# hammershock/SFM-Python

Hardware: AMD Instinct MI355X
Metric: BA iterations/sec (higher is better)
Workload: dtype f64

## Files before the change

sfm-python_amd/csrc/ba_kernels.hpp:

```cpp
#pragma once

#include <hip/hip_runtime.h>
#include <stdint.h>

#include "tr2d.hpp"

namespace sfmba {

constexpr int kCamTab = 17;
constexpr int kCamRow = 18;
#ifndef SFMBA_REC_LAYOUT
#define SFMBA_REC_LAYOUT 0
#endif
constexpr int kRecLayout = SFMBA_REC_LAYOUT;
constexpr int kRec = kRecLayout == 0 ? 6 : (kRecLayout == 1 ? 8 : 16);
constexpr int kVinvRow = kRecLayout == 0 ? 6 : (kRecLayout == 1 ? 8 : 16);
constexpr int kVinvInRec = kRecLayout == 2 ? 8 : -1;
constexpr int kRhsRec = 16;
constexpr int kSweepThreads = 1024;
constexpr int kWavesPerSweepBlock = kSweepThreads / 64;

struct KMat { double k[9]; };

constexpr int kJPlanes = 6;
// ... 2995 lines not shown
    }
    const size_t n6 = 6 * (size_t)C;
    const int set = ci.iters & 1;
    const double* __restrict__ vin = vecs + (size_t)set * kPcgVecs * n6;
    double* __restrict__ vout = vecs + (size_t)(set ^ 1) * kPcgVecs * n6;
    const double* __restrict__ u_in = vin + kPcgU * n6;
    const int slice = ((C + (int)gridDim.x - 1) / (int)gridDim.x + 63) & ~63;
    const int own_lo = (int)blockIdx.x * slice, own_hi = own_lo + slice;

    double d[1] = {0.0};
    for (int c = threadIdx.x; c < C; c += blockDim.x) {
#pragma unroll
        for (int k = 0; k < 6; ++k) {
            const size_t e = (size_t)k * C + c;
            const double ue = u_in[e];
            d[0] += (acc_in[e] + Dc[e] * ue) * ue;
        }
    }
    block_sum<1>(d, red);
    if (threadIdx.x == 0) sh_bcast[0] = d[0];
    __syncthreads();
    const double delta = sh_bcast[0];
    const double gamma = ci.rz;
    const double beta = ci.iters == 0 ? 0.0 : gamma / ci.rz_prev;
    const double den = delta - (ci.iters == 0 ? 0.0 : beta * gamma / ci.alpha_prev);
    const double alpha = gamma / den;
    if (!(den > 0.0) || !isfinite(alpha)) {
        if (blockIdx.x == 0 && threadIdx.x == 0) { PcgCtrl co = ci; co.done = 3; *cout = co; }
        return;
    }
    double t[1] = {0.0};
    for (int c = threadIdx.x; c < C; c += blockDim.x) {
        double rr[6], uu[6], pp[6], ss[6], xx[6], m[21];
#pragma unroll
        for (int n = 0; n < 21; ++n) m[n] = Minv[(size_t)n * C + c];
#pragma unroll
        for (int k = 0; k < 6; ++k) {
            const size_t e = (size_t)k * C + c;
            const double ue = u_in[e];
            const double we = acc_in[e] + Dc[e] * ue;
            pp[k] = ue + beta * vin[kPcgP * n6 + e];
            ss[k] = we + beta * vin[kPcgS * n6 + e];
            xx[k] = vin[kPcgX * n6 + e] + alpha * pp[k];
            rr[k] = vin[kPcgR * n6 + e] - alpha * ss[k];
        }
#pragma unroll
        for (int k = 0; k < 6; ++k) {
            uu[k] = minv_row(m, rr, k);
            t[0] += uu[k] * rr[k];
        }
        if (c >= own_lo && c < own_hi) {
#pragma unroll
            for (int k = 0; k < 6; ++k) {
                const size_t e = (size_t)k * C + c;
                vout[kPcgX * n6 + e] = xx[k]; vout[kPcgR * n6 + e] = rr[k];
                vout[kPcgP * n6 + e] = pp[k]; vout[kPcgS * n6 + e] = ss[k];
                vout[kPcgU * n6 + e] = uu[k];
                vout[kPcgUcm * n6 + 6 * (size_t)c + k] = uu[k];
            }
        }
    }
    block_sum<1>(t, red);
    if (blockIdx.x == 0 && threadIdx.x == 0) {
        PcgCtrl co = ci;
        co.rz_prev = ci.rz;
        co.alpha_prev = alpha;
        co.rz = t[0];
        co.iters = ci.iters + 1;
        if (!(t[0] > ci.tol2 * ci.rz0)) co.done = 1;
        else if (co.iters >= ci.max_iters) co.done = 2;
        *cout = co;
    }
}

constexpr int kBacksubCols = 10;
struct FinalUpdate {
    const double* __restrict__ part;
    double* __restrict__ vecs;
    PcgCtrl* __restrict__ ctrl2;
    int L;
};
template <bool LDS_VEC, bool JFREE = false>
__global__ __launch_bounds__(kSweepThreads) void k_backsub(
    const int2* __restrict__ ranges, int n_ranges, ObsArrays o, const double* __restrict__ dc_planes,
    double* __restrict__ dc, const double* __restrict__ Vinv, const double* __restrict__ gp,
    const double* __restrict__ t1, double* __restrict__ dp, double* __restrict__ part, int C,
    const PcgCtrl* __restrict__ ctrl2, int L, const double* __restrict__ gvec,
    const double* __restrict__ si, const double* __restrict__ sg, Recompute rc, FinalUpdate fu) {
    static_assert(!(LDS_VEC && JFREE), "J-free: the LDS holds the camera table, the step vector comes from L2");
    extern __shared__ __align__(16) double smem[];
    __shared__ double red[kBacksubCols * kWavesPerSweepBlock];
    if (LDS_VEC && fu.part != nullptr) {
        const int n6 = 6 * C, cam = threadIdx.x;
        const PcgCtrl ci = fu.ctrl2[fu.L & 1];
        PcgCtrl co = ci;
        double alpha = 0.0;
        double xe[6] = {0.0, 0.0, 0.0, 0.0, 0.0, 0.0}, pe[6] = {0.0, 0.0, 0.0, 0.0, 0.0, 0.0};
        if (cam < C) {
#pragma unroll
            for (int k = 0; k < 6; ++k) {
                xe[k] = fu.vecs[kPcgX * n6 + (size_t)k * C + cam];
                pe[k] = fu.vecs[kPcgP * n6 + (size_t)k * C + cam];
            }
        }
        if (ci.done == 0) alpha = pcg_local_step(fu.part, C, ci, co);
        if (blockIdx.x == 0 && threadIdx.x == 0) fu.ctrl2[(fu.L + 1) & 1] = co;
        if (co.done == 0) return;
        const bool add = ci.done == 0 && co.done != 3;
        if (cam < C) {
#pragma unroll
            for (int k = 0; k < 6; ++k) {
                const double xk = add ? xe[k] + alpha * pe[k] : xe[k];
                smem[6 * cam + k] = xk;
                if (blockIdx.x == 0) dc[6 * cam + k] = xk;
            }
        }
        __syncthreads();
    } else {
    if (ctrl2 != nullptr)
        dc_planes += (size_t)((ctrl2[L & 1].iters & 1) * kPcgVecs + kPcgX) * 6 * C;
    if (LDS_VEC) {
        for (int i = threadIdx.x; i < 6 * C; i += blockDim.x) {
            const int k = i / C, c = i - k * C;
            const double val = dc_planes[i];
            smem[6 * c + k] = val;
            if (blockIdx.x == 0) dc[6 * c + k] = val;
        }
        __syncthreads();
    }
    }
    if (JFREE) stage_cam_table(rc.camtab, C, smem);
    const double* __restrict__ vv = LDS_VEC ? smem : dc;
    const int wg = blockIdx.x * (blockDim.x >> 6) + (threadIdx.x >> 6);
    const int lane = threadIdx.x & 63;
    int pos = 0, end = 0;
    if (wg < n_ranges) { const int2 rg = ranges[wg]; pos = rg.x; end = rg.y; }
    auto blocks_of = [&](int j, int pj, double* jc_, double* jp_) {
        if (JFREE) recompute_blocks(rc, smem, o.cam_idx[j], pj, jc_, jp_);
        else load_blocks(o, j, jc_, jp_);
    };
    double g12 = 0.0, g22 = 0.0;
    double qs[8] = {0.0, 0.0, 0.0, 0.0, 0.0, 0.0, 0.0, 0.0};
    auto dots = [&](double* q, size_t e, double pe) {
        const double s = si[e];
        q[0] += gvec[e] * pe; q[1] += (pe * s) * (pe * s); q[2] += sg[e] * pe; q[3] += pe * pe;
    };

    auto jcv = [&](const double* jc, int c, double& t0, double& t1v) {
        const double2* a2 = reinterpret_cast<const double2*>(vv + 6 * c);
        const double2 a01 = a2[0], a23 = a2[1], a45 = a2[2];
        const double a[6] = {a01.x, a01.y, a23.x, a23.y, a45.x, a45.y};
        t0 = 0.0; t1v = 0.0;
#pragma unroll
        for (int k = 0; k < 6; ++k) { t0 += jc[k] * a[k]; t1v += jc[6 + k] * a[k]; }
    };
    auto point_dots = [&](int p, const double* s3, double z0, double z1, double z2) {
        const double z[3] = {z0, z1, z2};
#pragma unroll
        for (int k = 0; k < 3; ++k) {
            const double s_ = s3[k], ge = gp[3 * (size_t)p + k], pe = z[k];
            qs[0] += ge * pe; qs[1] += (pe * s_) * (pe * s_); qs[2] += (ge / (s_ * s_)) * pe; qs[3] += pe * pe;
        }
    };
    auto solve_point = [&](int p, const double* y, double& z0, double& z1, double& z2) {
        const double* vi = Vinv + kVinvRow * (size_t)p;
        const double b0 = -gp[3 * (size_t)p] - y[0], b1 = -gp[3 * (size_t)p + 1] - y[1],
                     b2 = -gp[3 * (size_t)p + 2] - y[2];
        z0 = vi[0] * b0 + vi[1] * b1 + vi[2] * b2;
        z1 = vi[1] * b0 + vi[3] * b1 + vi[4] * b2;
        z2 = vi[2] * b0 + vi[4] * b1 + vi[5] * b2;
        dp[3 * (size_t)p] = z0; dp[3 * (size_t)p + 1] = z1; dp[3 * (size_t)p + 2] = z2;
    };
    auto gram = [&](int i, const double* jp, double t0, double t1v, double z0, double z1, double z2) {
        const double a0 = t0 + jp[0] * z0 + jp[1] * z1 + jp[2] * z2;
        const double a1 = t1v + jp[3] * z0 + jp[4] * z1 + jp[5] * z2;
        const double2 tt = load_pair(t1, o.f32, i);
        g12 += tt.x * a0 + tt.y * a1;
        g22 += a0 * a0 + a1 * a1;
    };

    while (pos < end) {
        const int i = pos + lane;
        const bool in = i < end;
        const int p = in ? o.pt_idx[i] : o.pt_idx[pos];
        const int sb = o.pt_ptr[p], se = o.pt_ptr[p + 1];
        const bool complete = in && (se <= pos + 64);
        const int n_take = __popcll(__ballot(complete));
        double jc[12], jp[6];
        if (n_take == 0) {
            const int run_end = __shfl(se, 0);
            const int pp = __shfl(p, 0);
            double y[3] = {0.0, 0.0, 0.0};
            for (int j = pos + lane; j < run_end; j += 64) {
                blocks_of(j, pp, jc, jp);
                double t0, t1v;
                jcv(jc, o.cam_idx[j], t0, t1v);
                y[0] += jp[0] * t0 + jp[3] * t1v; y[1] += jp[1] * t0 + jp[4] * t1v;
                y[2] += jp[2] * t0 + jp[5] * t1v;
            }
            y[0] = wave_sum(y[0]); y[1] = wave_sum(y[1]); y[2] = wave_sum(y[2]);
            double z0, z1, z2;
            solve_point(pp, y, z0, z1, z2);
            if (lane == 0) point_dots(pp, si + 6 * (size_t)C + 3 * (size_t)pp, z0, z1, z2);
            for (int j = pos + lane; j < run_end; j += 64) {
                blocks_of(j, pp, jc, jp);
                double t0, t1v;
                jcv(jc, o.cam_idx[j], t0, t1v);
                gram(j, jp, t0, t1v, z0, z1, z2);
            }
            pos = run_end;
            continue;
        }
        const bool act = lane < n_take;
        double t0 = 0.0, t1v = 0.0, z0 = 0.0, z1 = 0.0, z2 = 0.0;
        double y[3] = {0.0, 0.0, 0.0};
        double s3[3] = {1.0, 1.0, 1.0};
        if (act) {
            blocks_of(i, p, jc, jp);
#pragma unroll
            for (int k = 0; k < 3; ++k) s3[k] = si[6 * (size_t)C + 3 * (size_t)p + k];
            jcv(jc, o.cam_idx[i], t0, t1v);
            y[0] = jp[0] * t0 + jp[3] * t1v; y[1] = jp[1] * t0 + jp[4] * t1v;
            y[2] = jp[2] * t0 + jp[5] * t1v;
        }
        seg_reduce_serial<3>(y, act ? sb : -1 - lane, lane);
        if (act && i == sb) { solve_point(p, y, z0, z1, z2); point_dots(p, s3, z0, z1, z2); }
        const int head = act ? lane - (i - sb) : lane;
        z0 = __shfl(z0, head); z1 = __shfl(z1, head); z2 = __shfl(z2, head);
        if (act) gram(i, jp, t0, t1v, z0, z1, z2);
        pos += n_take;
    }
    {
        const int per = (6 * C + (int)gridDim.x - 1) / (int)gridDim.x;
        const int e = (int)blockIdx.x * per + (int)threadIdx.x;
        if ((int)threadIdx.x < per && e < 6 * C) dots(qs + 4, (size_t)e, vv[e]);
    }
    double row[kBacksubCols];
    row[0] = wave_sum(g12);
    row[1] = wave_sum(g22);
#pragma unroll
    for (int k = 0; k < 8; ++k) row[2 + k] = wave_sum(qs[k]);
    if (lane == 0) {
#pragma unroll
        for (int k = 0; k < kBacksubCols; ++k) red[kBacksubCols * (threadIdx.x >> 6) + k] = row[k];
    }
    __syncthreads();
    if (threadIdx.x < kBacksubCols) {
        double a = 0.0;
        for (int w = 0; w < (int)(blockDim.x >> 6); ++w) a += red[kBacksubCols * w + threadIdx.x];
        part[(size_t)kBacksubCols * blockIdx.x + threadIdx.x] = a;
    }
}

__global__ void k_transpose(const double* __restrict__ in, int rows, int cols, double* __restrict__ out,
                            const PcgCtrl* __restrict__ ctrl2, int L) {
    const int i = blockIdx.x * blockDim.x + threadIdx.x;
    if (i >= rows * cols) return;
    if (ctrl2 != nullptr) in += (size_t)((ctrl2[L & 1].iters & 1) * kPcgVecs + kPcgX) * rows * cols;
    const int r = i / cols, c = i - r * cols;
    out[(size_t)c * rows + r] = in[i];
}

constexpr int kP2pMaxRanks = 16;
constexpr int kP2pFlagStride = 16;
constexpr int kP2pMaxBlocks = 32;
struct P2pArgs {
    double* data[kP2pMaxRanks];
    unsigned long long* flags[kP2pMaxRanks];
    int rank, world;
    long long stride;
    unsigned long long* seq;
    const int* cancel;
    unsigned* ticket;
    unsigned* error;
    long long timeout;
    unsigned long long max_mask;
    Piggyback rider;
    Mailbox post;
    const double* skip;
};

#ifdef SFMBA_P2P_NOFENCE
#ifndef SFMBA_EXPERIMENT
#error "SFMBA_P2P_NOFENCE builds collectives that are formally unordered: measurement builds only (-DSFMBA_EXPERIMENT)"
#endif
#define P2P_FENCE() asm volatile("s_waitcnt vmcnt(0) lgkmcnt(0)" ::: "memory")
#else
#define P2P_FENCE() __threadfence_system()
#endif
__device__ __forceinline__ unsigned p2p_take_ticket(unsigned* ticket) {
    return __hip_atomic_fetch_add(ticket, 1u, __ATOMIC_ACQ_REL, __HIP_MEMORY_SCOPE_AGENT);
}
__device__ __forceinline__ void p2p_allreduce_body(double* __restrict__ vec, int count, int op, const P2pArgs& a) {
    __shared__ unsigned s_last;
    const int tid = threadIdx.x;
    const unsigned long long seq = *a.seq + 1ull;
    const int par = (int)(seq & 1ull);
    const int per = (count + (int)gridDim.x - 1) / (int)gridDim.x;
    const int lo = (int)blockIdx.x * per, hi = min(count, lo + per);
    for (int q = 0; q < a.world; ++q) {
        double* dst = a.data[q] + ((size_t)par * a.world + a.rank) * a.stride;
        for (int e = lo + tid; e < hi; e += blockDim.x)
            __hip_atomic_store(dst + e, vec[e], __ATOMIC_RELAXED, __HIP_MEMORY_SCOPE_SYSTEM);
    }
    P2P_FENCE();
    __syncthreads();
    if (tid == 0) s_last = (p2p_take_ticket(a.ticket) == gridDim.x - 1) ? 1u : 0u;
    __syncthreads();
    if (s_last != 0u) {
        if (tid < a.world)
            __hip_atomic_store(a.flags[tid] + ((size_t)par * a.world + a.rank) * kP2pFlagStride, seq,
                               __ATOMIC_RELEASE, __HIP_MEMORY_SCOPE_SYSTEM);
        if (tid == 0) { *a.ticket = 0u; *a.seq = seq; }
// ... 156 lines not shown
```

sfm-python_amd/csrc/sfmba.hip:

```cpp
#include "../../include/sfmba.h"

#include <hip/hip_runtime.h>
#include <hip/hip_ext.h>
#include <rccl/rccl.h>
#include <dlfcn.h>

#include <algorithm>
#include <atomic>
#include <chrono>
#include <cmath>
#include <cstdarg>
#include <cstdio>
#include <cstdlib>
#include <cstring>
#include <condition_variable>
#include <functional>
#include <mutex>
#include <numeric>
#include <string>
#include <thread>
#include <vector>

#include "ba_kernels.hpp"
#include "tr2d.hpp"
// ... 96 lines not shown
            std::function<void(int)>* f = nullptr;
            {
                std::unique_lock<std::mutex> lk(m_);
                cv_.wait(lk, [&] { return gen_ != seen; });
                seen = gen_;
                if (stop_) return;
                if (id >= job_parts_ || job_ == nullptr) continue;
                f = job_;
            }
            (*f)(id);
            {
                std::lock_guard<std::mutex> lk(m_);
                if (--pending_ == 0) done_.notify_one();
            }
        }
    }
    std::vector<std::thread> th_;
    std::mutex m_;
    std::condition_variable cv_, done_;
    std::function<void(int)>* job_ = nullptr;
    int job_parts_ = 0, pending_ = 0;
    unsigned long long gen_ = 0;
    bool stop_ = false;
};

struct RcclApi {
    void* lib = nullptr;
    ncclResult_t (*GetUniqueId)(ncclUniqueId*) = nullptr;
    ncclResult_t (*CommInitRank)(ncclComm_t*, int, ncclUniqueId, int) = nullptr;
    ncclResult_t (*AllReduce)(const void*, void*, size_t, ncclDataType_t, ncclRedOp_t, ncclComm_t, hipStream_t) = nullptr;
    ncclResult_t (*CommDestroy)(ncclComm_t) = nullptr;
    const char* (*GetErrorString)(ncclResult_t) = nullptr;
};
RcclApi* rccl_api() {
    static RcclApi api;
    static bool tried = false;
    if (!tried) {
        tried = true;
        void* lib = dlopen("librccl.so.1", RTLD_NOW | RTLD_GLOBAL);
        if (!lib) lib = dlopen("librccl.so", RTLD_NOW | RTLD_GLOBAL);
        if (!lib) lib = dlopen("/opt/rocm/lib/librccl.so.1", RTLD_NOW | RTLD_GLOBAL);
        if (lib) {
            api.GetUniqueId = (decltype(api.GetUniqueId))dlsym(lib, "ncclGetUniqueId");
            api.CommInitRank = (decltype(api.CommInitRank))dlsym(lib, "ncclCommInitRank");
            api.AllReduce = (decltype(api.AllReduce))dlsym(lib, "ncclAllReduce");
            api.CommDestroy = (decltype(api.CommDestroy))dlsym(lib, "ncclCommDestroy");
            api.GetErrorString = (decltype(api.GetErrorString))dlsym(lib, "ncclGetErrorString");
            if (api.GetUniqueId && api.CommInitRank && api.AllReduce && api.CommDestroy && api.GetErrorString)
                api.lib = lib;
        }
    }
    return api.lib ? &api : nullptr;
}

double now_s() {
    return std::chrono::duration<double>(std::chrono::steady_clock::now().time_since_epoch()).count();
}

}

struct sfmba_handle {
    int device = 0;
    hipStream_t stream = nullptr;
    bool own_stream = false;
    std::string err;
    int n_cu = 256;

    bool have_problem = false;
    int64_t C = 0, P = 0, N = 0, ld = 0, n = 0;
    int64_t N_total = 0;
    KMat K{};
    bool permuted = false;
    std::vector<int64_t> order;
    int n_ranges = 0;
    bool f32 = false;
    bool f32_next = false;
    std::vector<int64_t> fixed_next;
    int64_t n_fixed = 0;
    bool lds_tab = true, lds_vec = true;
    bool sweep_rc = false;
    bool sweep_rc_g = false;
    DevBuf rctab;
    bool jfree = false;
    bool mixed = false;
    bool mixed_b = false;
    DevBuf rt32, rec32, rctab32, rtd;
    Origin origin{0.0, 0.0, 0.0};
    bool dense = false;
    DevView cov_ptr, cov_pt, blk_ab;
    DevBuf Sblk;
    DevBuf tables;
    int n_blk = 0;
    struct Debug {
        int pcg_fused = -1;
        int tab_lds = -1, vec_lds = -1;
        int sweep_rc = -1;
        int dense = -1;
        int precond = -1;
        int pcg_local = -1;
        int xcd_chunks = -1;
        int rhsrec = -1;
        int cost_rider = -1;
        int packed_upload = -1;
        int jfree = -1;
        int cm_device = -1;
        int pcg_inline = -1;
        int xcd_cam = -1;
        int pcg_skip_last = -1;
        int pcg_mixed_b = -1;
        int pcg_mixed = -1;
        int pcg_split = -1;
        int cam_chunk = 0;
        int pcg_guess_bias = 0;
        int trace_pcg = 0, trace_stalls = 0, trace_timing = 0;
        int wait_deadline_s = 120;
        int p2p_delay_ms = 0;
        int p2p_timeout_ms = 0;
    } dbg;

    DevBuf cam_idx, pt_idx, pt_ptr, uv;
    DevView ranges, wsteps, steps;
    int n_steps = 0;
    DevBuf cm_perm, cm_pt, cm_uv, cam_partial;
    DevBuf sort_hist, fixed_dev;
    DevView cam_ptr_dev;
    DevView cam_chunks, cam_chunk_ptr;
    int n_chunks = 0;
    DevView cam_chunks_b, cam_chunk_ptr_b;
    int n_chunks_b = 0;
    bool xcd_b = false;
    std::vector<int4> host_chunks_b;
    std::vector<int> host_chunk_ptr_b;
    bool cam_multi = false;
    DevBuf xa, xb, tabA, tabB, r, J, t1;
    DevBuf rhsrec;
    DevBuf V, Vinv, gp, e, recA, recB;
    DevBuf edge;
    DevBuf g, si, sg, p;
    DevBuf Dc, Minv, vecs, vtmp, vcm;
    DevBuf part, ctrl;
    DevBuf arena_own;
    double* arena = nullptr;
    int64_t arena_doubles = 0;
    sfmba_allreduce_fn ar_fn = nullptr;
    void* ar_ctx = nullptr;
    sfmba_print_fn print_fn = nullptr;
    void* print_ctx = nullptr;
    ncclComm_t comm = nullptr;
    int64_t n_collectives = 0, n_launches = 0;
    struct P2p {
        bool ready = false;
        int rank = 0, world = 0;
        int64_t stride = 0;
        void* own = nullptr;
        void* opened[kP2pMaxRanks] = {};
        double* data[kP2pMaxRanks] = {};
        unsigned long long* flags[kP2pMaxRanks] = {};
        double* camdata[kP2pMaxRanks] = {};
        unsigned* words = nullptr;
        int64_t calls = 0;
        bool first_in_solve = true;
        int shared_device = 1;
        bool any_multi = false;
    } p2p;
    double* h_scal = nullptr;
    struct Stage { PinnedBuf uv, ci, pi, perm, ptr, uvf, tables, ci16, uv16; } stage;
// ... 577 lines not shown
    }
    CamExchange cx{};
    if (cam_inline(h)) { cx = cam_exchange(h); ++h->p2p.calls; ++h->n_collectives; }
    if (xcd_cam(h)) {
        const CamMajor cmb{h->cam_chunks_b.as<int4>(), h->cm_pt.as<int>(), h->cm_uv.as<double>()};
        const int wgrid = h->n_chunks_b / kWaveChunkCams;
        const double* rr = h->use_rhsrec ? (const double*)h->rhsrec.as<double>() : (const double*)nullptr;
        if (h->f32 && !h->sweep_rc && !h->sweep_rc_g)
            hipLaunchKernelGGL((k_cam_rhs_diag_w<true>), dim3(wgrid), dim3(kCamThreads), 0, h->stream, cmb, (const double*)h->tab,
                               (const double*)h->rec, (const double*)vinv_ptr(h), h->K, h->cam_partial.as<double>(), rr);
        else
            hipLaunchKernelGGL((k_cam_rhs_diag_w<false>), dim3(wgrid), dim3(kCamThreads), 0, h->stream, cmb, (const double*)h->tab,
                               (const double*)h->rec, (const double*)vinv_ptr(h), h->K, h->cam_partial.as<double>(), rr);
        LAUNCHED(h);
        hipLaunchKernelGGL(k_cam_combine_w<27>, dim3((unsigned)((27 * C + 255) / 256)), dim3(256), 0, h->stream,
                           (const double*)h->cam_partial.as<double>(), (int)C, h->acc(), 1, (int)C, (const int*)nullptr,
                           (const double*)nullptr);
        LAUNCHED(h);
        CHK(exchange(h, h->acc(), 27 * C, 0));
        hipLaunchKernelGGL(k_cam_prep_schur, dim3((unsigned)((C + 63) / 64)), dim3(64), 0, h->stream, (const double*)h->Ugc(),
                           (const double*)h->sd(), (int)C, h->Dc.as<double>(), h->Minv.as<double>());
        LAUNCHED(h);
        return 0;
    }
    const bool own_inverse = !h->cam_multi && (!multi_rank(h) || cam_inline(h));
    const RhsPrecond mp = own_inverse ? RhsPrecond{h->Ugc(), h->Dc.as<double>(), h->Minv.as<double>()} : RhsPrecond{nullptr, nullptr, nullptr};
    if (h->f32 && !h->sweep_rc && !h->sweep_rc_g)
        hipLaunchKernelGGL((k_cam_rhs_diag<true>), dim3(h->n_chunks), dim3(kRhsThreads), 0, h->stream, cam_major(h),
                           (const double*)h->tab, (const double*)h->rec, (const double*)vinv_ptr(h), h->K, (int)C,
                           h->acc(), h->cam_partial.as<double>(), mp, h->use_rhsrec ? (const double*)h->rhsrec.as<double>() : (const double*)nullptr, cx);
    else
        hipLaunchKernelGGL((k_cam_rhs_diag<false>), dim3(h->n_chunks), dim3(kRhsThreads), 0, h->stream, cam_major(h),
                           (const double*)h->tab, (const double*)h->rec, (const double*)vinv_ptr(h), h->K, (int)C,
                           h->acc(), h->cam_partial.as<double>(), mp, h->use_rhsrec ? (const double*)h->rhsrec.as<double>() : (const double*)nullptr, cx);
    LAUNCHED(h);
    if (own_inverse) return 0;
    CHK(launch_cam_combine(h, 27, h->acc(), 1, (int)C, nullptr, nullptr));
    CHK(exchange(h, h->acc(), 27 * C, 0));
    hipLaunchKernelGGL(k_cam_prep_schur, dim3((unsigned)((C + 63) / 64)), dim3(64), 0, h->stream, (const double*)h->Ugc(),
                       (const double*)h->sd(), (int)C, h->Dc.as<double>(), h->Minv.as<double>());
    LAUNCHED(h);
    return 0;
}

constexpr double kDenseTolFactor = 0.1;
int launch_dense_solve(sfmba_handle* h, double tol, int max_iters, bool rhs) {
    hipLaunchKernelGGL(k_schur_blocks, dim3(h->n_blk), dim3(kCamThreads), 0, h->stream, (const int*)h->cov_ptr.as<int>(),
                       (const int*)h->cov_pt.as<int>(), (const int2*)h->blk_ab.as<int2>(), (const double*)h->tab,
                       (const double*)h->rec, (const double*)vinv_ptr(h), h->K, (int)h->C,
                       h->Sblk.as<double>(), rhs ? h->acc() : (double*)nullptr);
    LAUNCHED(h);
    const int n = 6 * (int)h->C;
    const size_t lds = sizeof(double) * ((size_t)n * (size_t)(n | 1) + 2 * kDenseMaxN + ((21 * kDenseMaxN / 6 + 1) & ~1) +
                                         4 * (kDenseThreads / 64));
    CHK(set_lds(h, k_dense_pcg, lds));
    hipLaunchKernelGGL(k_dense_pcg, dim3(1), dim3(kDenseThreads), lds, h->stream, (const double*)h->Sblk.as<double>(),
                       (const double*)h->Ugc(), (const double*)h->Dc.as<double>(),
                       (const double*)h->acc(), (int)h->C, tol, max_iters, h->vecs.as<double>(), h->ctrl.as<PcgCtrl>());
    LAUNCHED(h);
    h->pcg_L = 0;
    return 0;
}

int schur_product_standalone(sfmba_handle* h, const double* v_planes) {
    const double* va = v_planes;
    if (!h->lds_vec && !h->sweep_rc && !h->sweep_rc_g) {
        hipLaunchKernelGGL(k_transpose, dim3((unsigned)((6 * h->C + 255) / 256)), dim3(256), 0, h->stream, v_planes,
                           6, (int)h->C, h->vcm.as<double>(), (const PcgCtrl*)nullptr, 0);
        LAUNCHED(h);
        va = h->vcm.as<double>();
    }
    CHK(launch_point_sweep(h, va, nullptr, 0));
    return launch_cam_schur<0>(h, v_planes, nullptr, 0);
}

int launch_jdot(sfmba_handle* h, int* nparts) {
    const int grid = grid_1d(h->N, kSweepThreads, h->n_cu);
    const double* sgc = h->sg.as<double>();
    const double* sgp = sgc + 6 * h->C;
    Piggyback pb{};
    if (h->pending_scale_sums) pb = slices_rider(h, 0, 4);
    const int launch_grid = grid + (pb.part != nullptr ? 1 : 0);
    const Recompute rc{h->tab, h->x + 6 * h->C, h->K};
    if (h->jfree) {
        const size_t lds = sizeof(double) * kCamRow * (size_t)h->C;
        auto kern = k_jdot<false, true>;
        CHK(set_lds(h, kern, lds));
        hipLaunchKernelGGL(kern, dim3(launch_grid), dim3(kSweepThreads), lds, h->stream, obs_arrays(h), sgc, sgp,
                           (int)h->N, (int)h->C, h->t1.as<double>(), h->partB(), pb, rc);
    } else if (h->lds_vec) {
        const size_t lds = sizeof(double) * 6 * h->C;
        auto kern = k_jdot<true>;
        CHK(set_lds(h, kern, lds));
        hipLaunchKernelGGL(kern, dim3(launch_grid), dim3(kSweepThreads), lds, h->stream, obs_arrays(h), sgc, sgp,
                           (int)h->N, (int)h->C, h->t1.as<double>(), h->partB(), pb, rc);
    } else {
        hipLaunchKernelGGL(k_jdot<false>, dim3(launch_grid), dim3(kSweepThreads), 0, h->stream, obs_arrays(h),
                           sgc, sgp, (int)h->N, (int)h->C, h->t1.as<double>(), h->partB(), pb, rc);
    }
    LAUNCHED(h);
    h->pending_scale_sums = false;
    *nparts = grid;
    return 0;
}

int launch_backsub(sfmba_handle* h, int* nparts) {
    const int grid = (h->n_ranges + kWavesPerSweepBlock - 1) / kWavesPerSweepBlock;
    double* dc = h->p.as<double>();
    double* dp = dc + 6 * h->C;
    const PcgCtrl* ctrl2 = h->ctrl.as<PcgCtrl>();
    const Recompute rc{h->tab, h->x + 6 * h->C, h->K};
    if (h->jfree) {
        hipLaunchKernelGGL(k_transpose, dim3((6 * h->C + 255) / 256), dim3(256), 0, h->stream,
                           (const double*)h->vecs.as<double>(), 6, (int)h->C, dc, ctrl2, h->pcg_L);
        LAUNCHED(h);
        const size_t lds = sizeof(double) * kCamRow * (size_t)h->C;
        auto kern = k_backsub<false, true>;
        CHK(set_lds(h, kern, lds));
        hipLaunchKernelGGL(kern, dim3(grid), dim3(kSweepThreads), lds, h->stream, h->ranges.as<int2>(), h->n_ranges, obs_arrays(h),
                           h->vecs.as<double>(), dc, vinv_ptr(h), h->gp.as<double>(), h->t1.as<double>(), dp, h->partB(),
                           (int)h->C, (const PcgCtrl*)nullptr, 0, h->g.as<double>(), h->si.as<double>(), h->sg.as<double>(), rc, FinalUpdate{});
    } else if (h->lds_vec) {
        const size_t lds = sizeof(double) * 6 * h->C;
        auto kern = k_backsub<true>;
        CHK(set_lds(h, kern, lds));
        hipLaunchKernelGGL(kern, dim3(grid), dim3(kSweepThreads), lds, h->stream, h->ranges.as<int2>(),
                           h->n_ranges, obs_arrays(h), h->vecs.as<double>(), dc, vinv_ptr(h),
                           h->gp.as<double>(), h->t1.as<double>(), dp, h->partB(), (int)h->C,
                           ctrl2, h->pcg_L, h->g.as<double>(), h->si.as<double>(), h->sg.as<double>(), rc,
                           h->pcg_a_owed ? FinalUpdate{h->pcg_part.as<double>(), h->vecs.as<double>(), h->ctrl.as<PcgCtrl>(), h->pcg_L - 1}
                                         : FinalUpdate{});
    } else {
        hipLaunchKernelGGL(k_transpose, dim3((6 * h->C + 255) / 256), dim3(256), 0, h->stream,
                           (const double*)h->vecs.as<double>(), 6, (int)h->C, dc, ctrl2, h->pcg_L);
        LAUNCHED(h);
        hipLaunchKernelGGL(k_backsub<false>, dim3(grid), dim3(kSweepThreads), 0, h->stream,
                           h->ranges.as<int2>(), h->n_ranges, obs_arrays(h), h->vecs.as<double>(), dc,
                           vinv_ptr(h), h->gp.as<double>(), h->t1.as<double>(), dp,
                           h->partB(), (int)h->C, (const PcgCtrl*)nullptr, 0, h->g.as<double>(),
                           h->si.as<double>(), h->sg.as<double>(), rc, FinalUpdate{});
    }
    LAUNCHED(h);
    *nparts = grid;
    return 0;
}

int launch_update_scale(sfmba_handle* h, int first, bool defer = false) {
    if (h->scale_pts == 2)
        hipLaunchKernelGGL(k_update_scale<2>, dim3(h->red_grid), dim3(256), 0, h->stream, h->Ugc(), h->V.as<double>(),
                           h->gp.as<double>(), h->x, (int)h->C, (int)h->P, first, h->red_bc, h->si.as<double>(),
                           h->g.as<double>(), h->sg.as<double>(), h->part.as<double>());
    else
        hipLaunchKernelGGL(k_update_scale<1>, dim3(h->red_grid), dim3(256), 0, h->stream, h->Ugc(), h->V.as<double>(),
                           h->gp.as<double>(), h->x, (int)h->C, (int)h->P, first, h->red_bc, h->si.as<double>(),
                           h->g.as<double>(), h->sg.as<double>(), h->part.as<double>());
    LAUNCHED(h);
    if (defer) { h->pending_scale_sums = true; return 0; }
    return launch_finish_slices(h, 0, 4);
}

Piggyback backsub_rider(sfmba_handle* h, int nparts) {
    Piggyback pb{h->partB(), h->scal(), FinishJob{}, 1, kBacksubCols, 0};
    pb.job.row0[0] = 0; pb.job.nrows[0] = nparts;
    for (int k = 0; k < kFinishCols; ++k) { pb.job.slot[0][k] = -1; pb.job.slot[1][k] = -1; }
    for (int k = 0; k < 6; ++k) pb.job.slot[0][k] = 2 + k;
    for (int k = 0; k < 4; ++k) pb.job.slot[0][6 + k] = kCamSlot + 5 + k;
    return pb;
}
int launch_finish_backsub(sfmba_handle* h, int nparts) {
    const Piggyback pb = backsub_rider(h, nparts);
    hipLaunchKernelGGL(k_finish, dim3(1), dim3(64 * kBacksubCols), 0, h->stream, pb.part, pb.job, kBacksubCols, 0,
                       h->scal(), (const double*)nullptr, Mailbox{});
    LAUNCHED(h);
    return 0;
}

int flush_scale_sums(sfmba_handle* h) {
    if (!h->pending_scale_sums) return 0;
    h->pending_scale_sums = false;
    return launch_finish_slices(h, 0, 4);
}
int exchange_linearise(sfmba_handle* h) {
    CHK(exchange(h, h->scal() + 8, 4, 0));
    CHK(exchange(h, h->scal() + kMaxSlot, 1, 1));
    return 0;
}
int exchange_tail(sfmba_handle* h) {
    return exchange(h, h->scal() + 2, 6, 0);
}

int fetch_scalars(sfmba_handle* h) {
    const Mailbox mb{h->mbox_dev, h->scal(), nullptr, ++h->mbox_seq, p2p_error_word(h)};
    hipLaunchKernelGGL(k_post, dim3(1), dim3(64), 0, h->stream, mb);
    LAUNCHED(h);
    CHK(wait_mailbox(h, h->mbox_seq));
    memcpy(h->h_scal, h->mbox, sizeof(double) * kScalSlots);
    return 0;
}

double qsum(const sfmba_handle* h, int q) { return h->h_scal[kPointSlot[q]] + h->h_scal[kCamSlot + q]; }

int ensure_h_x(sfmba_handle* h) {
    const size_t need = (size_t)std::max<int64_t>(h->n, 2 * h->N);
    if (h->h_x && h->h_x_doubles >= need) return 0;
    if (h->h_x) { (void)hipHostFree(h->h_x); h->h_x = nullptr; h->h_x_doubles = 0; }
    HIPCHK(h, hipHostMalloc((void**)&h->h_x, sizeof(double) * need, hipHostMallocDefault));
    h->h_x_doubles = need;
    return 0;
}

template <class Fn>
void staging_copy(sfmba_handle* h, void* dst, const void* src, size_t bytes, Fn chunk_done) {
    const int parts = (int)std::min<size_t>(4, bytes >> 19);
    if (parts <= 1) { memcpy(dst, src, bytes); chunk_done(0, (size_t)0, bytes); return; }
    const size_t per = ((bytes + parts - 1) / parts + 63) & ~(size_t)63;
    std::atomic<int> done[8];
    for (auto& d : done) d.store(0, std::memory_order_relaxed);
    h->pool.run(parts, [&](int t) {
        const size_t b = std::min(bytes, (size_t)t * per), e = std::min(bytes, b + per);
        if (e > b) memcpy(static_cast<char*>(dst) + b, static_cast<const char*>(src) + b, e - b);
// ... 818 lines not shown
        h->xcd_b = h->dbg.xcd_chunks == 1 || (h->dbg.xcd_chunks != 0 && P >= 250000);
        if (h->xcd_b) {
            constexpr int kX = kWaveChunkRanges, kG = kWaveChunkCams;
            static_assert(kX == 8, "one range per XCD");
            const int64_t groups = (C + kG - 1) / kG;
            chunks_b.assign((size_t)(groups * kX * kG), make_int4(-1, 0, 0, kX));
            for (int64_t c = 0; c < C && !cm_device; ++c) {
                const int b = cam_ptr[c], e = cam_ptr[c + 1];
                int prev = b;
                for (int k = 0; k < kX; ++k) {
                    int bound = e;
                    if (k + 1 < kX) {
                        const int64_t p_hi = P * (int64_t)(k + 1) / kX;
                        int lo = prev, hi = e;
                        while (lo < hi) { const int mid = (lo + hi) >> 1; if (pi[perm[mid]] < p_hi) lo = mid + 1; else hi = mid; }
                        bound = lo;
                    }
                    chunks_b[(size_t)(((c / kG) * kX + k) * kG + c % kG)] = make_int4((int)c, prev, bound, kX);
                    prev = bound;
                }
            }
        }
        h->n_chunks_b = (int)chunks_b.size();
    }
    h->dense = 6 * C <= kDenseMaxN && h->dbg.dense != 0;
    std::vector<int> cov_ptr, cov_pt;
    std::vector<int2> blk_ab;
    if (h->dense) {
        const int nblk = (int)(C * (C + 1) / 2);
        cov_ptr.assign((size_t)nblk + 1, 0);
        const int pp = P >= 32768 ? 4 : 1;
        std::vector<int> cnt((size_t)pp * (size_t)nblk, 0);
        const int64_t pper = (P + pp - 1) / pp;
        auto each_pair = [&](int t, auto&& visit) {
            const int64_t p0 = std::min<int64_t>(P, t * pper), p1 = std::min<int64_t>(P, p0 + pper);
            for (int64_t p = p0; p < p1; ++p)
                for (int i = ptr[p]; i < ptr[p + 1]; ++i)
                    for (int j = i; j < ptr[p + 1]; ++j) {
                        const int a = std::min(ci[i], ci[j]), b = std::max(ci[i], ci[j]);
                        if (fixed[(size_t)a] || fixed[(size_t)b]) continue;
                        visit((int)p, dense_block_index(a, b, (int)C), i == j, a == b);
                    }
        };
        h->pool.run(pp, [&](int t) {
            int* ct = cnt.data() + (size_t)t * (size_t)nblk;
            each_pair(t, [&](int, int blk, bool self, bool same_cam) { ct[blk] += (self || !same_cam) ? 1 : 2; });
        });
        int64_t total = 0;
        for (int blk = 0; blk < nblk; ++blk) {
            cov_ptr[(size_t)blk] = (int)std::min<int64_t>(total, INT32_MAX);
            for (int t = 0; t < pp; ++t) { int& v = cnt[(size_t)t * (size_t)nblk + blk]; const int n_e = v; v = (int)std::min<int64_t>(total, INT32_MAX); total += n_e; }
        }
        cov_ptr[(size_t)nblk] = (int)std::min<int64_t>(total, INT32_MAX);
        if (total > ((int64_t)1 << 26)) h->dense = false;
        else {
            cov_pt.resize((size_t)std::max<int64_t>(1, total));
            h->pool.run(pp, [&](int t) {
                int* fill = cnt.data() + (size_t)t * (size_t)nblk;
                each_pair(t, [&](int p, int blk, bool self, bool same_cam) {
                    int& f = fill[blk];
                    cov_pt[(size_t)f++] = self ? ~p : p;
                    if (!self && same_cam) cov_pt[(size_t)f++] = p;
                });
            });
            blk_ab.resize((size_t)nblk);
            for (int a = 0; a < (int)C; ++a)
                for (int b = a; b < (int)C; ++b) blk_ab[(size_t)dense_block_index(a, b, (int)C)] = make_int2(a, b);
            h->n_blk = nblk;
        }
    }
    tp2 = now_s();
    h->lds_tab = (size_t)C * kCamRow * sizeof(double) <= kLdsDynMax;
    h->lds_vec = (size_t)C * 6 * sizeof(double) <= kLdsDynMax;
    if (h->dbg.tab_lds == 0) h->lds_tab = false;
    if (h->dbg.vec_lds == 0) h->lds_vec = false;
    h->sweep_rc = C <= kRcMaxCams && (size_t)C * kRcRow * sizeof(double) <= kLdsDynMax && h->dbg.sweep_rc != 0 &&
                  h->dbg.sweep_rc != 2;
    h->sweep_rc_g = !h->sweep_rc && h->dbg.sweep_rc != 0;
    h->pcg_fused = (h->lds_vec || h->sweep_rc) && C <= kSweepThreads;
    if (h->dbg.pcg_fused == 0) h->pcg_fused = false;
    h->mixed = (h->sweep_rc || h->sweep_rc_g) && (h->dbg.pcg_mixed == 1 || (h->dbg.pcg_mixed != 0 && f32));
    h->mixed_b = h->mixed && h->dbg.pcg_mixed_b != 0;
    h->jfree = h->dbg.jfree == 1 && h->lds_tab;

    const size_t esz = f32 ? sizeof(float) : sizeof(double);
    const size_t keep = (size_t)fdiff;
    HIPCHK(h, h->cam_idx.ensure_keep(sizeof(int) * ldz, sizeof(int) * keep));
    HIPCHK(h, h->pt_idx.ensure_keep(sizeof(int) * ldz, sizeof(int) * keep));
    HIPCHK(h, h->uv.ensure_keep(esz * 2 * ldz, esz * 2 * keep));
    const int64_t p_keep = keep == 0 ? 0 : std::min<int64_t>(std::min<int64_t>(prev.P, P), (int64_t)pi[fdiff - 1] + 1);
    HIPCHK(h, h->pt_ptr.ensure_keep(sizeof(int) * ((size_t)P + 1), sizeof(int) * (size_t)p_keep));
    struct Piece { const void* src; size_t bytes; DevView* view; size_t off; };
    Piece pieces[11] = {
        {cam_ptr.data(), sizeof(int) * cam_ptr.size(), &h->cam_ptr_dev, 0},
        {ranges.data(), sizeof(int2) * ranges.size(), &h->ranges, 0}, {wsteps.data(), sizeof(int2) * wsteps.size(), &h->wsteps, 0},
        {steps.data(), sizeof(int2) * steps.size(), &h->steps, 0}, {chunks.data(), sizeof(int4) * chunks.size(), &h->cam_chunks, 0},
        {chunk_ptr.data(), sizeof(int) * chunk_ptr.size(), &h->cam_chunk_ptr, 0},
        {cov_ptr.data(), h->dense ? sizeof(int) * cov_ptr.size() : 0, &h->cov_ptr, 0},
        {cov_pt.data(), h->dense ? sizeof(int) * cov_pt.size() : 0, &h->cov_pt, 0},
        {blk_ab.data(), h->dense ? sizeof(int2) * blk_ab.size() : 0, &h->blk_ab, 0},
        {h->host_chunks_b.data(), sizeof(int4) * h->host_chunks_b.size(), &h->cam_chunks_b, 0},
        {h->host_chunk_ptr_b.data(), sizeof(int) * h->host_chunk_ptr_b.size(), &h->cam_chunk_ptr_b, 0}};
    size_t tables_bytes = 0;
    for (auto& pc : pieces) { pc.off = tables_bytes; tables_bytes += (pc.bytes + 255) / 256 * 256; }
    HIPCHK(h, h->tables.ensure(tables_bytes + 256));
    HIPCHK(h, sg.tables.ensure(tables_bytes + 256, 0));
    for (auto& pc : pieces) {
        if (pc.bytes) memcpy(sg.tables.as<char>() + pc.off, pc.src, pc.bytes);
        pc.view->p = h->tables.as<char>() + pc.off;
    }
    HIPCHK(h, h->xa.ensure(sizeof(double) * h->n));
    HIPCHK(h, h->xb.ensure(sizeof(double) * h->n));
    HIPCHK(h, h->tabA.ensure(sizeof(double) * cam_table_doubles((int)C)));
    HIPCHK(h, h->tabB.ensure(sizeof(double) * cam_table_doubles((int)C)));
    HIPCHK(h, h->r.ensure(esz * 2 * ldz));
    HIPCHK(h, h->J.ensure(esz * 12 * ldz));
    HIPCHK(h, h->cm_perm.ensure(sizeof(int) * ldz));
    HIPCHK(h, h->cm_pt.ensure(sizeof(int) * ldz));
    HIPCHK(h, h->cm_uv.ensure(esz * 2 * ldz));
    HIPCHK(h, h->cam_partial.ensure(sizeof(double) * std::max<size_t>(27 * chunks.size(), 27 * h->host_chunks_b.size())));
    HIPCHK(h, h->recA.ensure(sizeof(double) * kRec * P));
    HIPCHK(h, h->recB.ensure(sizeof(double) * kRec * P));
    h->use_rhsrec = h->dbg.rhsrec == 1 || (h->dbg.rhsrec != 0 && P >= 250000);
    if (h->use_rhsrec) HIPCHK(h, h->rhsrec.ensure(sizeof(double) * kRhsRec * P));
    if (h->dense) {
        HIPCHK(h, h->Sblk.ensure(sizeof(double) * 36 * blk_ab.size()));
    }
    HIPCHK(h, h->t1.ensure(esz * 2 * ldz));
    HIPCHK(h, h->V.ensure(sizeof(double) * 6 * P));
    HIPCHK(h, h->Vinv.ensure(sizeof(double) * (kVinvInRec < 0 ? kVinvRow * P : 8)));
    HIPCHK(h, h->gp.ensure(sizeof(double) * 3 * P + 16));
    HIPCHK(h, h->edge.ensure(sizeof(double) * 2 * kEdgeRow * (size_t)((N + 63) / 64)));
    HIPCHK(h, h->e.ensure(sizeof(double) * 3 * P));
    HIPCHK(h, h->g.ensure(sizeof(double) * h->n));
    HIPCHK(h, h->si.ensure(sizeof(double) * h->n));
    HIPCHK(h, h->sg.ensure(sizeof(double) * h->n));
    HIPCHK(h, h->p.ensure(sizeof(double) * h->n + 16));
    HIPCHK(h, h->Dc.ensure(sizeof(double) * 6 * C));
    HIPCHK(h, h->Minv.ensure(sizeof(double) * 21 * C));
    HIPCHK(h, h->vecs.ensure(sizeof(double) * 2 * kPcgVecs * 6 * C));
    HIPCHK(h, h->vtmp.ensure(sizeof(double) * 6 * C));
    HIPCHK(h, h->vcm.ensure(sizeof(double) * 6 * C));
    if (h->sweep_rc_g) HIPCHK(h, h->rctab.ensure(sizeof(double) * kRcRow * (size_t)C));
    if (h->mixed) {
        HIPCHK(h, h->rt32.ensure(sizeof(float) * kRt32 * (size_t)C));
        HIPCHK(h, h->rtd.ensure(sizeof(double) * kRt32 * (size_t)C));
        HIPCHK(h, h->rec32.ensure(sizeof(float) * kRec32 * (size_t)P));
        if (h->sweep_rc_g) HIPCHK(h, h->rctab32.ensure(sizeof(float) * kRc32Row * (size_t)C));
    }
    h->scale_pts = P >= 65536 ? 2 : 1;
    h->red_bc = grid_1d(6 * C, 256, 32);
    h->red_grid = h->red_bc + grid_1d(P, 256 * h->scale_pts, 992);
    HIPCHK(h, h->part.ensure(sizeof(double) * (size_t)(2 * kPartRows * kNQ)));
    HIPCHK(h, h->ctrl.ensure(2 * sizeof(PcgCtrl)));
    HIPCHK(h, h->pcg_part.ensure(sizeof(double) * 4 * C));
    HIPCHK(h, h->arena_own.ensure(sizeof(double) * (size_t)sfmba_exchange_doubles(C)));
    h->arena = h->arena_own.as<double>();
    h->ar_fn = nullptr; h->ar_ctx = nullptr;
    h->x = h->xa.as<double>(); h->x_new = h->xb.as<double>();
    h->tab = h->tabA.as<double>(); h->tab_new = h->tabB.as<double>();
    h->rec = h->recA.as<double>(); h->rec_new = h->recB.as<double>();

    auto up = [&](void* dst, const void* src, size_t elem, size_t from, size_t to) -> hipError_t {
        if (to <= from) return hipSuccess;
        return hipMemcpyAsync(static_cast<char*>(dst) + elem * from, static_cast<const char*>(src) + elem * from,
                              elem * (to - from), hipMemcpyHostToDevice, h->stream);
// ... 719 lines not shown
```

Before: 2562.

## Drive backsub sweep from precomputed step table with prefetched indices; enable recompute jdot in f64

The backsub kernel now walks a precomputed per-wave step table instead of discovering point-complete segments at runtime with ballots and pt_ptr lookups. Step descriptors and camera/point indices are prefetched two to three steps ahead, and the first loads are issued before the PCG step and the sync. Per-point data such as Vinv, gp and t1 is loaded per lane, and segment heads are found with a ballot. Separately, a new jdot_rc flag turns on the Jacobian-recompute jdot kernel for f64 whenever the camera table fits in LDS. This adds register pressure and changes the f64 default path.

Result: no change. 2566 (median of 4 runs) (+0.2%).

```diff
diff --git a/sfm-python_amd/csrc/ba_kernels.hpp b/sfm-python_amd/csrc/ba_kernels.hpp
--- a/sfm-python_amd/csrc/ba_kernels.hpp
+++ b/sfm-python_amd/csrc/ba_kernels.hpp
@@ -3101,7 +3101,7 @@
 };
 template <bool LDS_VEC, bool JFREE = false>
 __global__ __launch_bounds__(kSweepThreads) void k_backsub(
-    const int2* __restrict__ ranges, int n_ranges, ObsArrays o, const double* __restrict__ dc_planes,
+    StepTable st, ObsArrays o, const double* __restrict__ dc_planes,
     double* __restrict__ dc, const double* __restrict__ Vinv, const double* __restrict__ gp,
     const double* __restrict__ t1, double* __restrict__ dp, double* __restrict__ part, int C,
     const PcgCtrl* __restrict__ ctrl2, int L, const double* __restrict__ gvec,
@@ -3109,6 +3109,26 @@
     static_assert(!(LDS_VEC && JFREE), "J-free: the LDS holds the camera table, the step vector comes from L2");
     extern __shared__ __align__(16) double smem[];
     __shared__ double red[kBacksubCols * kWavesPerSweepBlock];
+    const int wg = blockIdx.x * (blockDim.x >> 6) + (threadIdx.x >> 6);
+    const int lane = threadIdx.x & 63;
+    int2 wv = make_int2(0, 0);
+    if (wg < st.n_waves) wv = st.wsteps[wg];
+    int s = 0, s_end = 0;
+    int2 cur = make_int2(0, 0), nxt = make_int2(0, 0), nn = make_int2(0, 0);
+    int c = 0, p = 0, cn = 0, pn = 0;
+    auto request_steps = [&]() {
+        s = __builtin_amdgcn_readfirstlane(wv.x); s_end = s + __builtin_amdgcn_readfirstlane(wv.y);
+        if (s < s_end) cur = st.steps[s];
+        if (s + 1 < s_end) nxt = st.steps[s + 1];
+        if (s + 2 < s_end) nn = st.steps[s + 2];
+    };
+    auto request_indices = [&]() {
+        cur.x = __builtin_amdgcn_readfirstlane(cur.x); cur.y = __builtin_amdgcn_readfirstlane(cur.y);
+        nxt.x = __builtin_amdgcn_readfirstlane(nxt.x); nxt.y = __builtin_amdgcn_readfirstlane(nxt.y);
+        nn.x = __builtin_amdgcn_readfirstlane(nn.x); nn.y = __builtin_amdgcn_readfirstlane(nn.y);
+        if (cur.y <= 64 && lane < cur.y) { c = o.cam_idx[cur.x + lane]; p = o.pt_idx[cur.x + lane]; }
+        if (nxt.y <= 64 && lane < nxt.y) { cn = o.cam_idx[nxt.x + lane]; pn = o.pt_idx[nxt.x + lane]; }
+    };
     if (LDS_VEC && fu.part != nullptr) {
         const int n6 = 6 * C, cam = threadIdx.x;
         const PcgCtrl ci = fu.ctrl2[fu.L & 1];
@@ -3122,9 +3142,11 @@
                 pe[k] = fu.vecs[kPcgP * n6 + (size_t)k * C + cam];
             }
         }
+        request_steps();
         if (ci.done == 0) alpha = pcg_local_step(fu.part, C, ci, co);
         if (blockIdx.x == 0 && threadIdx.x == 0) fu.ctrl2[(fu.L + 1) & 1] = co;
         if (co.done == 0) return;
+        request_indices();
         const bool add = ci.done == 0 && co.done != 3;
         if (cam < C) {
 #pragma unroll
@@ -3136,8 +3158,10 @@
         }
         __syncthreads();
     } else {
+    request_steps();
     if (ctrl2 != nullptr)
         dc_planes += (size_t)((ctrl2[L & 1].iters & 1) * kPcgVecs + kPcgX) * 6 * C;
+    request_indices();
     if (LDS_VEC) {
         for (int i = threadIdx.x; i < 6 * C; i += blockDim.x) {
             const int k = i / C, c = i - k * C;
@@ -3150,12 +3174,8 @@
     }
     if (JFREE) stage_cam_table(rc.camtab, C, smem);
     const double* __restrict__ vv = LDS_VEC ? smem : dc;
-    const int wg = blockIdx.x * (blockDim.x >> 6) + (threadIdx.x >> 6);
-    const int lane = threadIdx.x & 63;
-    int pos = 0, end = 0;
-    if (wg < n_ranges) { const int2 rg = ranges[wg]; pos = rg.x; end = rg.y; }
-    auto blocks_of = [&](int j, int pj, double* jc_, double* jp_) {
-        if (JFREE) recompute_blocks(rc, smem, o.cam_idx[j], pj, jc_, jp_);
+    auto blocks_of = [&](int j, int cj, int pj, double* jc_, double* jp_) {
+        if (JFREE) recompute_blocks(rc, smem, cj, pj, jc_, jp_);
         else load_blocks(o, j, jc_, jp_);
     };
     double g12 = 0.0, g22 = 0.0;
@@ -3173,81 +3193,92 @@
 #pragma unroll
         for (int k = 0; k < 6; ++k) { t0 += jc[k] * a[k]; t1v += jc[6 + k] * a[k]; }
     };
-    auto point_dots = [&](int p, const double* s3, double z0, double z1, double z2) {
+    auto point_dots = [&](const double* g3, const double* s3, double z0, double z1, double z2) {
         const double z[3] = {z0, z1, z2};
 #pragma unroll
         for (int k = 0; k < 3; ++k) {
-            const double s_ = s3[k], ge = gp[3 * (size_t)p + k], pe = z[k];
+            const double s_ = s3[k], ge = g3[k], pe = z[k];
             qs[0] += ge * pe; qs[1] += (pe * s_) * (pe * s_); qs[2] += (ge / (s_ * s_)) * pe; qs[3] += pe * pe;
         }
     };
-    auto solve_point = [&](int p, const double* y, double& z0, double& z1, double& z2) {
-        const double* vi = Vinv + kVinvRow * (size_t)p;
-        const double b0 = -gp[3 * (size_t)p] - y[0], b1 = -gp[3 * (size_t)p + 1] - y[1],
-                     b2 = -gp[3 * (size_t)p + 2] - y[2];
+    auto solve_point = [&](int p, const double* vi, const double* g3, const double* y, double& z0, double& z1, double& z2) {
+        const double b0 = -g3[0] - y[0], b1 = -g3[1] - y[1], b2 = -g3[2] - y[2];
         z0 = vi[0] * b0 + vi[1] * b1 + vi[2] * b2;
         z1 = vi[1] * b0 + vi[3] * b1 + vi[4] * b2;
         z2 = vi[2] * b0 + vi[4] * b1 + vi[5] * b2;
         dp[3 * (size_t)p] = z0; dp[3 * (size_t)p + 1] = z1; dp[3 * (size_t)p + 2] = z2;
     };
-    auto gram = [&](int i, const double* jp, double t0, double t1v, double z0, double z1, double z2) {
+    auto gram = [&](double2 tt, const double* jp, double t0, double t1v, double z0, double z1, double z2) {
         const double a0 = t0 + jp[0] * z0 + jp[1] * z1 + jp[2] * z2;
         const double a1 = t1v + jp[3] * z0 + jp[4] * z1 + jp[5] * z2;
-        const double2 tt = load_pair(t1, o.f32, i);
         g12 += tt.x * a0 + tt.y * a1;
         g22 += a0 * a0 + a1 * a1;
     };
 
-    while (pos < end) {
-        const int i = pos + lane;
-        const bool in = i < end;
-        const int p = in ? o.pt_idx[i] : o.pt_idx[pos];
-        const int sb = o.pt_ptr[p], se = o.pt_ptr[p + 1];
-        const bool complete = in && (se <= pos + 64);
-        const int n_take = __popcll(__ballot(complete));
+    while (s < s_end) {
+        int2 n3 = make_int2(0, 0);
+        if (s + 3 < s_end) n3 = st.steps[s + 3];
+        int c2 = 0, p2 = 0;
+        if (nn.y <= 64 && lane < nn.y) { c2 = o.cam_idx[nn.x + lane]; p2 = o.pt_idx[nn.x + lane]; }
         double jc[12], jp[6];
-        if (n_take == 0) {
-            const int run_end = __shfl(se, 0);
-            const int pp = __shfl(p, 0);
+        if (cur.y > 64) {
+            const int run_end = cur.x + cur.y;
+            const int pp = o.pt_idx[cur.x];
             double y[3] = {0.0, 0.0, 0.0};
-            for (int j = pos + lane; j < run_end; j += 64) {
-                blocks_of(j, pp, jc, jp);
+            for (int j = cur.x + lane; j < run_end; j += 64) {
+                const int cj = o.cam_idx[j];
+                blocks_of(j, cj, pp, jc, jp);
                 double t0, t1v;
-                jcv(jc, o.cam_idx[j], t0, t1v);
+                jcv(jc, cj, t0, t1v);
                 y[0] += jp[0] * t0 + jp[3] * t1v; y[1] += jp[1] * t0 + jp[4] * t1v;
                 y[2] += jp[2] * t0 + jp[5] * t1v;
             }
             y[0] = wave_sum(y[0]); y[1] = wave_sum(y[1]); y[2] = wave_sum(y[2]);
             double z0, z1, z2;
-            solve_point(pp, y, z0, z1, z2);
-            if (lane == 0) point_dots(pp, si + 6 * (size_t)C + 3 * (size_t)pp, z0, z1, z2);
-            for (int j = pos + lane; j < run_end; j += 64) {
-                blocks_of(j, pp, jc, jp);
+            solve_point(pp, Vinv + kVinvRow * (size_t)pp, gp + 3 * (size_t)pp, y, z0, z1, z2);
+            if (lane == 0) point_dots(gp + 3 * (size_t)pp, si + 6 * (size_t)C + 3 * (size_t)pp, z0, z1, z2);
+            for (int j = cur.x + lane; j < run_end; j += 64) {
+                const int cj = o.cam_idx[j];
+                blocks_of(j, cj, pp, jc, jp);
                 double t0, t1v;
-                jcv(jc, o.cam_idx[j], t0, t1v);
-                gram(j, jp, t0, t1v, z0, z1, z2);
-            }
-            pos = run_end;
-            continue;
-        }
-        const bool act = lane < n_take;
-        double t0 = 0.0, t1v = 0.0, z0 = 0.0, z1 = 0.0, z2 = 0.0;
-        double y[3] = {0.0, 0.0, 0.0};
-        double s3[3] = {1.0, 1.0, 1.0};
-        if (act) {
-            blocks_of(i, p, jc, jp);
-#pragma unroll
-            for (int k = 0; k < 3; ++k) s3[k] = si[6 * (size_t)C + 3 * (size_t)p + k];
-            jcv(jc, o.cam_idx[i], t0, t1v);
-            y[0] = jp[0] * t0 + jp[3] * t1v; y[1] = jp[1] * t0 + jp[4] * t1v;
-            y[2] = jp[2] * t0 + jp[5] * t1v;
-        }
-        seg_reduce_serial<3>(y, act ? sb : -1 - lane, lane);
-        if (act && i == sb) { solve_point(p, y, z0, z1, z2); point_dots(p, s3, z0, z1, z2); }
-        const int head = act ? lane - (i - sb) : lane;
-        z0 = __shfl(z0, head); z1 = __shfl(z1, head); z2 = __shfl(z2, head);
-        if (act) gram(i, jp, t0, t1v, z0, z1, z2);
-        pos += n_take;
+                jcv(jc, cj, t0, t1v);
+                gram(load_pair(t1, o.f32, j), jp, t0, t1v, z0, z1, z2);
+            }
+        } else {
+            const int i = cur.x + lane;
+            const bool act = lane < cur.y;
+            double t0 = 0.0, t1v = 0.0, z0 = 0.0, z1 = 0.0, z2 = 0.0;
+            double y[3] = {0.0, 0.0, 0.0};
+            double s3[3] = {1.0, 1.0, 1.0}, g3[3] = {0.0, 0.0, 0.0}, vi[6] = {0.0, 0.0, 0.0, 0.0, 0.0, 0.0};
+            double2 tt = make_double2(0.0, 0.0);
+            if (act) {
+                blocks_of(i, c, p, jc, jp);
+#pragma unroll
+                for (int k = 0; k < 3; ++k) s3[k] = si[6 * (size_t)C + 3 * (size_t)p + k];
+#pragma unroll
+                for (int k = 0; k < 3; ++k) g3[k] = gp[3 * (size_t)p + k];
+#pragma unroll
+                for (int k = 0; k < 6; ++k) vi[k] = Vinv[kVinvRow * (size_t)p + k];
+                tt = load_pair(t1, o.f32, i);
+                jcv(jc, c, t0, t1v);
+                y[0] = jp[0] * t0 + jp[3] * t1v; y[1] = jp[1] * t0 + jp[4] * t1v;
+                y[2] = jp[2] * t0 + jp[5] * t1v;
+            }
+            const int key = act ? p : -1 - lane;
+            seg_reduce_serial<3>(y, key, lane);
+            const int prev = lane_below(key, lane);
+            const bool is_head = act && (lane == 0 || prev != key);
+            if (is_head) { solve_point(p, vi, g3, y, z0, z1, z2); point_dots(g3, s3, z0, z1, z2); }
+            const unsigned long long heads = __ballot(is_head);
+            const int head = act ? 63 - __clzll((long long)(heads & (~0ull >> (63 - lane)))) : lane;
+            z0 = __shfl(z0, head); z1 = __shfl(z1, head); z2 = __shfl(z2, head);
+            if (act) gram(tt, jp, t0, t1v, z0, z1, z2);
+        }
+        cur = nxt; nxt = nn;
+        nn.x = __builtin_amdgcn_readfirstlane(n3.x);
+        nn.y = __builtin_amdgcn_readfirstlane(n3.y);
+        c = cn; p = pn; cn = c2; pn = p2;
+        ++s;
     }
     {
         const int per = (6 * C + (int)gridDim.x - 1) / (int)gridDim.x;
diff --git a/sfm-python_amd/csrc/sfmba.hip b/sfm-python_amd/csrc/sfmba.hip
--- a/sfm-python_amd/csrc/sfmba.hip
+++ b/sfm-python_amd/csrc/sfmba.hip
@@ -202,6 +202,7 @@
     bool sweep_rc_g = false;
     DevBuf rctab;
     bool jfree = false;
+    bool jdot_rc = false;
     bool mixed = false;
     bool mixed_b = false;
     DevBuf rt32, rec32, rctab32, rtd;
@@ -945,7 +946,7 @@
     if (h->pending_scale_sums) pb = slices_rider(h, 0, 4);
     const int launch_grid = grid + (pb.part != nullptr ? 1 : 0);
     const Recompute rc{h->tab, h->x + 6 * h->C, h->K};
-    if (h->jfree) {
+    if (h->jdot_rc) {
         const size_t lds = sizeof(double) * kCamRow * (size_t)h->C;
         auto kern = k_jdot<false, true>;
         CHK(set_lds(h, kern, lds));
@@ -980,15 +981,14 @@
         const size_t lds = sizeof(double) * kCamRow * (size_t)h->C;
         auto kern = k_backsub<false, true>;
         CHK(set_lds(h, kern, lds));
-        hipLaunchKernelGGL(kern, dim3(grid), dim3(kSweepThreads), lds, h->stream, h->ranges.as<int2>(), h->n_ranges, obs_arrays(h),
+        hipLaunchKernelGGL(kern, dim3(grid), dim3(kSweepThreads), lds, h->stream, step_table(h), obs_arrays(h),
                            h->vecs.as<double>(), dc, vinv_ptr(h), h->gp.as<double>(), h->t1.as<double>(), dp, h->partB(),
                            (int)h->C, (const PcgCtrl*)nullptr, 0, h->g.as<double>(), h->si.as<double>(), h->sg.as<double>(), rc, FinalUpdate{});
     } else if (h->lds_vec) {
         const size_t lds = sizeof(double) * 6 * h->C;
         auto kern = k_backsub<true>;
         CHK(set_lds(h, kern, lds));
-        hipLaunchKernelGGL(kern, dim3(grid), dim3(kSweepThreads), lds, h->stream, h->ranges.as<int2>(),
-                           h->n_ranges, obs_arrays(h), h->vecs.as<double>(), dc, vinv_ptr(h),
+        hipLaunchKernelGGL(kern, dim3(grid), dim3(kSweepThreads), lds, h->stream, step_table(h), obs_arrays(h), h->vecs.as<double>(), dc, vinv_ptr(h),
                            h->gp.as<double>(), h->t1.as<double>(), dp, h->partB(), (int)h->C,
                            ctrl2, h->pcg_L, h->g.as<double>(), h->si.as<double>(), h->sg.as<double>(), rc,
                            h->pcg_a_owed ? FinalUpdate{h->pcg_part.as<double>(), h->vecs.as<double>(), h->ctrl.as<PcgCtrl>(), h->pcg_L - 1}
@@ -998,7 +998,7 @@
                            (const double*)h->vecs.as<double>(), 6, (int)h->C, dc, ctrl2, h->pcg_L);
         LAUNCHED(h);
         hipLaunchKernelGGL(k_backsub<false>, dim3(grid), dim3(kSweepThreads), 0, h->stream,
-                           h->ranges.as<int2>(), h->n_ranges, obs_arrays(h), h->vecs.as<double>(), dc,
+                           step_table(h), obs_arrays(h), h->vecs.as<double>(), dc,
                            vinv_ptr(h), h->gp.as<double>(), h->t1.as<double>(), dp,
                            h->partB(), (int)h->C, (const PcgCtrl*)nullptr, 0, h->g.as<double>(),
                            h->si.as<double>(), h->sg.as<double>(), rc, FinalUpdate{});
@@ -1983,6 +1983,7 @@
     h->mixed = (h->sweep_rc || h->sweep_rc_g) && (h->dbg.pcg_mixed == 1 || (h->dbg.pcg_mixed != 0 && f32));
     h->mixed_b = h->mixed && h->dbg.pcg_mixed_b != 0;
     h->jfree = h->dbg.jfree == 1 && h->lds_tab;
+    h->jdot_rc = h->jfree || (!f32 && h->lds_tab);
 
     const size_t esz = f32 ? sizeof(float) : sizeof(double);
     const size_t keep = (size_t)fdiff;
```
